# gbbin/DDP-practice

Hardware: AMD Instinct MI355X
Metric: images/sec (whole node) + 3-epoch wall-clock, MNIST ConvNet at 1/2/4/8 MI355X (higher is better)
Workload: dtype bf16; 1 GPU; model=ConvNet (2x[Conv5x5-BN-ReLU-MaxPool2] + Linear(1568,10), 29,034 params), global_batch=32, parallelism=dp1, per_rank_batch=32, impl=native (fused HIP kernels, C++ reducer/communicator), sync_bn=False, amp=autocast bf16 + GradScaler, optimizer=SGD(lr=1e-4), hipgraph=True, steps_per_graph=16, comm=none (1 rank), grad_avg=none (1 rank)

## Files before the change

ddp_practice_amd/csrc/kernels/convblock_impl.h:

```cpp
#pragma once
#include "common.h"
#include "comm/xsite.h"

namespace dpa {
namespace cb {

constexpr int NTHR = 256;

__host__ __device__ constexpr int stats_len(int C) { return 3 * C + 1; }
__host__ __device__ constexpr int fslab_row(int C) { return 2 * C + 1; }

template <int I> struct SH;
template <> struct SH<0> { static constexpr int CIN = 1, COUT = 16, H = 28, W = 28, SPLIT = 4, WROWS = 28; };
#ifndef DPA_FWD2_SPLIT
#define DPA_FWD2_SPLIT 2
#endif
template <> struct SH<1> { static constexpr int CIN = 16, COUT = 32, H = 14, W = 14, SPLIT = DPA_FWD2_SPLIT, WROWS = 14; };
constexpr int kBwdSplit = 8;

template <int N, typename Sink>
__device__ __forceinline__ void stage_f32(const float* __restrict__ src, Sink&& sink) {
  static_assert(N % 4 == 0, "N must be a multiple of 4");
  constexpr int N4 = N / 4;
  constexpr int IT = (N4 + NTHR - 1) / NTHR;
  f32x4 v[IT];
  const f32x4* s4 = reinterpret_cast<const f32x4*>(src);
#pragma unroll
  for (int i = 0; i < IT; ++i) {
    const int e = threadIdx.x + i * NTHR;
    if (e < N4) v[i] = s4[e];
  }
#pragma unroll
  for (int i = 0; i < IT; ++i) {
    const int e = threadIdx.x + i * NTHR;
    if (e < N4) {
#pragma unroll
      for (int j = 0; j < 4; ++j) sink(4 * e + j, v[i][j]);
    }
  }
}

template <typename T> struct Pair2 { typedef uint32_t type; };
template <> struct Pair2<float> { typedef uint64_t type; };
template <typename T, int C, int H, int W, typename Sink>
__device__ __forceinline__ void stage_chw(const T* __restrict__ src, Sink&& sink) {
  static_assert(W % 2 == 0, "W must be even");
  typedef typename Pair2<T>::type P;
  constexpr int NP = C * H * W / 2;
  constexpr int IT = (NP + NTHR - 1) / NTHR;
  P v[IT];
  const P* s2 = reinterpret_cast<const P*>(src);
#pragma unroll
  for (int i = 0; i < IT; ++i) {
    const int e = threadIdx.x + i * NTHR;
    if (e < NP) v[i] = s2[e];
  }
#pragma unroll
  for (int i = 0; i < IT; ++i) {
    const int e = threadIdx.x + i * NTHR;
    if (e < NP) {
      const int pe = 2 * e;
      const int c = pe / (H * W), rem = pe % (H * W);
      T a, b;
      __builtin_memcpy(&a, &v[i], sizeof(T));
      __builtin_memcpy(&b, reinterpret_cast<const char*>(&v[i]) + sizeof(T), sizeof(T));
      sink(c, rem / W, rem % W, a, b);
    }
  }
}

struct BNParams {
  const float* fslab;
  int nrows;
  float* fstats;
  const float* gamma;
  const float* beta;
  float* rmean;
  float* rvar;
  int64_t* nbt;
  float momentum;
  float eps;
  int train;
  xgmi::XSite xs;
};

constexpr int RSUM_U = 24;
template <typename F>
__device__ __forceinline__ float strided_rowsum(const float* __restrict__ src, int rows, int RL, int j, int g, int G,
                                                F&& after_issue) {
  float acc = 0.f;
  auto batch = [&](int base, bool first) {
    float v[RSUM_U];
#pragma unroll
    for (int u = 0; u < RSUM_U; ++u) {
      const int rr = base + u * G;
      v[u] = src[(size_t)min(rr, rows - 1) * RL + j] * (rr < rows ? 1.f : 0.f);
    }
    if (first) after_issue();
#pragma unroll
    for (int u = 0; u < RSUM_U; ++u) acc += v[u];
  };
  batch(g, true);
  for (int base = g + RSUM_U * G; base < rows; base += RSUM_U * G) batch(base, false);
  return acc;
}
__device__ __forceinline__ float strided_rowsum(const float* __restrict__ src, int rows, int RL, int j, int g, int G) {
  return strided_rowsum(src, rows, RL, j, g, G, [] {});
}

template <int C>
__device__ __forceinline__ void bn_finalize(const BNParams& bp, float* sc_s, float* beta_s, float* mean_s,
                                            float* istd_s, float* part, int bid) {
  const int tid = threadIdx.x, nthr = NTHR;
  const bool leader = bid == 0;
  if (bp.train) {
    constexpr int RL = 2 * C + 1;
    const int G = nthr / RL;
    const int j = tid % RL, g = tid / RL;
    float gam = 0.f, bet = 0.f, shf = 0.f, rm = 0.f, rv = 0.f;
    if (tid < C) {
      gam = bp.gamma[tid];
      bet = bp.beta[tid];
      shf = bp.fstats[2 * C + 1 + tid];
      if (leader) {
        rm = bp.rmean[tid];
        rv = bp.rvar[tid];
      }
    }
    const int64_t nb0 = leader ? bp.nbt[0] : 0;
    const bool xon = bp.xs.active();
    unsigned long long tk = 0;
    auto ticket = [&] {
      if (xon && tid == 0) tk = xgmi::xsite_ticket(bp.xs, bid);
    };
    if (g < G) {
      part[tid] = strided_rowsum(bp.fslab, bp.nrows, RL, j, g, G, ticket);
    } else {
      ticket();
      part[tid] = 0.f;
    }
    DPA_STAMP(11);
    __syncthreads();
    DPA_STAMP(12);
    if (tid < RL) {
      float t = 0.f;
      for (int gg = 0; gg < G; ++gg) t += part[gg * RL + tid];
      part[tid] = t;
    }
    __syncthreads();
    if (xon) xgmi::xsite_exchange(bp.xs, part, RL, tk, bid);
    if (tid < C) {
      const float n = part[2 * C];
      const float m1 = part[tid] / n;
      const float mean = shf + m1;
      const float var = fmaxf(part[C + tid] / n - m1 * m1, 0.f);
      const float istd = rsqrtf(var + bp.eps);
      const float s = gam * istd;
      sc_s[tid] = s;
      beta_s[tid] = bet;
      mean_s[tid] = mean;
      istd_s[tid] = istd;
      if (leader) {
        bp.fstats[tid] = part[tid];
        bp.fstats[C + tid] = part[C + tid];
        if (tid == 0) bp.fstats[2 * C] = n;
        const int64_t nb = nb0 + 1;
        const float mom = bp.momentum >= 0.f ? bp.momentum : 1.f / (float)nb;
        bp.rmean[tid] = (1.f - mom) * rm + mom * mean;
        bp.rvar[tid] = (1.f - mom) * rv + mom * var * (n / fmaxf(n - 1.f, 1.f));
      }
    }
    __syncthreads();
    if (leader && tid == 0) bp.nbt[0] = nb0 + 1;
  } else {
    if (tid < C) {
      const float istd = rsqrtf(bp.rvar[tid] + bp.eps);
      const float s = bp.gamma[tid] * istd;
      sc_s[tid] = s;
      beta_s[tid] = bp.beta[tid];
      mean_s[tid] = bp.rmean[tid];
      istd_s[tid] = istd;
    }
    __syncthreads();
  }
}

template <typename T>
__device__ __forceinline__ void bn_relu_max4x(const typename Pair2<T>::type top, const typename Pair2<T>::type bot,
                                              float sc, float beta, float mean, float istd, float& best, int& bi,
                                              float& xh) {
  T v[4];
  __builtin_memcpy(&v[0], &top, 2 * sizeof(T));
  __builtin_memcpy(&v[2], &bot, 2 * sizeof(T));
  best = -1.f;
  bi = 0;
  float yb = 0.f;
#pragma unroll
  for (int k = 0; k < 4; ++k) {
    const float yv = Cvt<T>::to_f(v[k]);
    const float z = fmaxf(rnd_t<T>((yv - mean) * sc + beta), 0.f);
    if (z > best) { best = z; bi = k; yb = yv; }
  }
  xh = (yb - mean) * istd;
}

constexpr int IDX_POS = 3, IDX_RELU = 4;

template <typename T>
struct PoolIn {
  const T* y;
  BNParams bn;
  T* p_out;
  uint8_t* idx_out;
  T* xh_out;
};

template <typename T>
struct BwdIn {
  const T* dp;
  const uint8_t* idx;
  const T* y;
  const float* fstats;
  const float* gsum;
  int grows;
  const float* lsum;
  int lrows;
  const float* gamma;
  float eps;
  float* dgamma;
  float* dbeta;
  xgmi::XSite xs;
  GradChk chk;
  int chk_coef = 0;
  int chk_rows = 0;
  float chk_row_bound = 0.f;
};

__device__ __forceinline__ void colsum_rows(const float* __restrict__ src, int rows, int RL, float* part,
                                            float* out) {
  const int tid = threadIdx.x, nthr = NTHR;
  const int G = nthr / RL;
  const int j = tid % RL, g = tid / RL;
  part[tid] = g < G ? strided_rowsum(src, rows, RL, j, g, G) : 0.f;
  __syncthreads();
  float t = 0.f;
  if (tid < RL)
    for (int gg = 0; gg < G; ++gg) t += part[gg * RL + tid];
  __syncthreads();
  if (tid < RL) out[tid] = t;
  __syncthreads();
}

template <int C, typename T>
__device__ __forceinline__ void bn_bwd_coef(const BwdIn<T>& bi, float* coef, float* part, float* sums, int bid) {
  const int tid = threadIdx.x;
  const bool leader = bid == 0;
  float n = 0.f, f0 = 0.f, f1 = 0.f, shf = 0.f, gam = 0.f;
  if (tid < C) {
    n = bi.fstats[2 * C];
    f0 = bi.fstats[tid];
    f1 = bi.fstats[C + tid];
    shf = bi.fstats[2 * C + 1 + tid];
    gam = bi.gamma[tid];
  }
  const bool xon = bi.xs.active();
  unsigned long long tk = 0;
  if (xon && tid == 0) tk = xgmi::xsite_ticket(bi.xs, bid);
  const bool cchk = leader && bi.dgamma != nullptr && bi.chk_coef && !xon;
  colsum_rows(bi.gsum, bi.grows, 2 * C, part, sums);
  if (xon) {
    if (leader && bi.dgamma != nullptr && tid < C) {
      bi.dgamma[tid] = sums[C + tid];
      bi.dbeta[tid] = sums[tid];
      if (bi.chk_coef) bi.chk.flag(GradChk::bad(sums[C + tid], bi.chk.bound) || GradChk::bad(sums[tid], bi.chk.bound));
    }
    xgmi::xsite_exchange(bi.xs, sums, 2 * C, tk, bid);
  }
  if (tid < C) {
    const float m1 = f0 / n;
    const float mean = shf + m1;
    const float istd = rsqrtf(fmaxf(f1 / n - m1 * m1, 0.f) + bi.eps);
    coef[tid] = sums[tid] / n;
    coef[C + tid] = sums[C + tid] / n;
    coef[2 * C + tid] = gam * istd;
    coef[3 * C + tid] = mean;
    coef[4 * C + tid] = istd;
    if (leader && bi.dgamma != nullptr && bi.lsum == bi.gsum && !xon) {
      bi.dgamma[tid] = sums[C + tid];
      bi.dbeta[tid] = sums[tid];
    }
  }
  __syncthreads();
  if (leader && bi.dgamma != nullptr && bi.lsum != bi.gsum && !xon) {
    colsum_rows(bi.lsum, bi.lrows, 2 * C, part, sums);
    if (tid < C) {
      bi.dgamma[tid] = sums[C + tid];
      bi.dbeta[tid] = sums[tid];
    }
  }
  if (cchk && tid < C)
    bi.chk.flag(GradChk::bad(sums[C + tid], bi.chk.bound) || GradChk::bad(sums[tid], bi.chk.bound));
}

template <typename T, int C, int H, int W, int NT_, int ROWS = H>
struct BnBwdStage {
  typedef typename Pair2<T>::type P;
  static_assert(ROWS % 2 == 0 && ROWS <= H, "BN-backward staging works on whole 2x2 pooling windows");
  static constexpr int HO = H / 2, WO = W / 2, PP = HO * WO;
  static constexpr int CHO = ROWS / 2, CPP = CHO * WO, NWIN = C * CPP;
  static constexpr int IT = (NWIN + NT_ - 1) / NT_;
// ... 214 lines not shown
      return px * CIN + c;
    } else {
      return px * CIN + ((((c >> 3) ^ ((px / PPB) & (NCH - 1)))) << 3) + (c & 7);
    }
  };
  __shared__ float lstat[(NTHR / 64) * 2 * COUT];

  const int tid = threadIdx.x;
  const int b = bid / nsplit;
  DPA_STAMP(0);
  const int sp = bid % nsplit;
  const T* xb = x + (size_t)b * CIN * HW;
  const int mt0 = (MT * sp) / nsplit, mt1 = (MT * (sp + 1)) / nsplit;
  float pre_bias[NT], pre_shift[NT];
#pragma unroll
  for (int nt = 0; nt < NT; ++nt) {
    const int co = nt * 16 + (tid & 15);
    pre_bias[nt] = (MODE == 2) ? 0.f : bias[co];
    pre_shift[nt] = (MODE == 0) ? shift[co] : 0.f;
  }

  const T zero = Cvt<T>::from_f(0.f);
  constexpr int WN16 = WPK == 1 ? COUT * KPW * (int)sizeof(T) / 16 : 1;
  constexpr int WIT = (WN16 + NTHR - 1) / NTHR;
  auto load_wpk = [&]() {
    if constexpr (WPK == 1) {
      static_assert((COUT * KPW * sizeof(T)) % 16 == 0, "packed weight tile must be whole 16-B chunks");
      static_assert(COUT * KPW == (MODE == 2 ? W2D_LEN : W2F_LEN), "pre-packed weights exist for layer 2 only");
      typedef __attribute__((address_space(3))) void* lds_ptr_t;
      const uint4* src = reinterpret_cast<const uint4*>(wpk);
      uint4* dstl = reinterpret_cast<uint4*>(wl);
      const int wv0 = (tid >> 6) * 64, ln = tid & 63;
#pragma unroll
      for (int i = 0; i < WIT; ++i) {
        const int c0 = i * NTHR + wv0;
        if (c0 + ln < WN16)
          __builtin_amdgcn_global_load_lds(src + c0 + ln, (lds_ptr_t)(dstl + c0), 16, 0, 0);
      }
    }
  };
  if constexpr (WPK == 1) {
    if constexpr (PRO == 0 || PRO == 3) load_wpk();
  } else {
    if constexpr (KP > K) {
      for (int e = tid; e < COUT * (KP - K); e += NTHR) wl[(e / (KP - K)) * KPW + K + e % (KP - K)] = zero;
    }
    constexpr int KO = 25 * (MODE == 2 ? COUT : CIN);
    stage_f32<COUT * K>(w, [&](int e, float v) {
      const int o = e / KO, rem = e % KO;
      const int i = rem / 25, tap = rem % 25;
      if (MODE == 2)
        wl[i * KPW + (24 - tap) * CIN + o] = Cvt<T>::from_f(v);
      else
        wl[o * KPW + tap * CIN + i] = Cvt<T>::from_f(v);
    });
  }
  if constexpr (WPK == 2) pack_w2<T>(pk);
  DPA_STAMP(1);
  if constexpr ((CIN * sizeof(T)) % 16 == 0) {
    constexpr int G = CIN * (int)sizeof(T) / 16;
    uint4* img4 = reinterpret_cast<uint4*>(img);
    for (int e = tid; e < HP * WPD * G; e += NTHR) {
      const int px = e / G, hp = px / WPD, wp = px % WPD;
      if (hp < 2 || hp >= H + 2 || wp < 2 || wp >= W + 2) img4[e] = make_uint4(0u, 0u, 0u, 0u);
    }
  } else {
    for (int e = tid; e < HP * WPD * CIN; e += NTHR) {
      const int hp = e / (WPD * CIN), rem = e % (WPD * CIN);
      const int wp = rem / CIN;
      if (hp < 2 || hp >= H + 2 || wp < 2 || wp >= W + 2) img[e] = zero;
    }
  }
  constexpr int EPIX = EPI ? MT * 16 : 1;
  __shared__ uint8_t eidx[EPI ? COUT * EPIX : 1];
  __shared__ T exh[EPI ? COUT * EPIX : 1];
  const int ep0 = mt0 * 16, enp = min(mt1 * 16, HW) - ep0;
  constexpr int EIT = EPI ? (COUT * EPIX + NTHR - 1) / NTHR : 1;
  uint8_t ei[EIT];
  T ex[EIT];
  auto load_epi = [&]() {
    if constexpr (EPI == 1) {
#pragma unroll
      for (int i = 0; i < EIT; ++i) {
        const int e = tid + i * NTHR;
        const int ec = e < COUT * enp ? e : 0;
        const int co = ec / enp, pp = ec % enp;
        const size_t o = ((size_t)b * COUT + co) * HW + ep0 + pp;
        ei[i] = epi.idx[o];
        ex[i] = epi.xh[o];
      }
    }
  };
  auto store_epi = [&]() {
    if constexpr (EPI == 1) {
#pragma unroll
      for (int i = 0; i < EIT; ++i) {
        const int e = tid + i * NTHR;
        if (e < COUT * enp) {
          const int co = e / enp, pp = e % enp;
          eidx[co * EPIX + pp] = ei[i];
          exh[co * EPIX + pp] = ex[i];
        }
      }
    }
  };
  if constexpr (PRO != 2) {
    load_epi();
    store_epi();
  }
  DPA_STAMP(2);
  constexpr int DQ = PRO != 1 ? 1
                     : (CIN % 8 == 0 && sizeof(T) == 2) ? 8 * ((CIN / 8 * HW + NTHR - 1) / NTHR)
                                                          : (CIN * HW + NTHR - 1) / NTHR;
  int dq_e[DQ];
  T dq_p[DQ], dq_x[DQ];
  uint8_t dq_i[DQ];
#pragma unroll
  for (int d = 0; d < DQ; ++d) dq_e[d] = -1;
  if constexpr (PRO == 0) {
    stage_chw<T, CIN, H, W>(xb, [&](int ci, int h, int ww, T a, T bb) {
      img[imo((h + 2) * WPD + (ww + 2), ci)] = a;
      img[imo((h + 2) * WPD + (ww + 3), ci)] = bb;
    });
  } else if constexpr (PRO == 3) {
    static_assert(HW % 4 == 0 && W % 4 == 0, "4-pixel groups stay inside a row");
    constexpr int G4 = HW / 4, GIT = (G4 + NTHR - 1) / NTHR;
    const int step = __builtin_amdgcn_readfirstlane(*reinterpret_cast<volatile int*>(gin.ctr));
    long long pos = (long long)step * gin.nimg + b;
    pos = pos < gin.order_len ? pos : gin.order_len - 1;
    const int64_t src = gin.order[pos];
    const uint32_t* s4 = reinterpret_cast<const uint32_t*>(gin.imgs + src * HW);
    uint32_t v4[GIT];
#pragma unroll
    for (int i = 0; i < GIT; ++i)
      if (tid + i * NTHR < G4) v4[i] = s4[tid + i * NTHR];
    if (sp == 0 && tid == 0) gin.lab_out[b] = gin.labels[src];
    T* xo = const_cast<T*>(xb);
#pragma unroll
    for (int i = 0; i < GIT; ++i) {
      const int g = tid + i * NTHR;
      if (g < G4) {
        const int h = (4 * g) / W, ww = (4 * g) % W;
        T px[4];
#pragma unroll
        for (int k = 0; k < 4; ++k) {
          px[k] = Cvt<T>::from_f((float)((v4[i] >> (8 * k)) & 0xffu) * gin.scale + gin.shift);
          img[imo((h + 2) * WPD + (ww + k + 2), 0)] = px[k];
        }
        if (sp == 0) {
#pragma unroll
          for (int k = 0; k < 4; ++k) xo[4 * g + k] = px[k];
        }
      }
    }
    if (tid == 0) {
      const int arrived = __hip_atomic_fetch_add(&gin.ctr[1], 1, __ATOMIC_RELAXED, __HIP_MEMORY_SCOPE_AGENT);
      if (arrived == gin.nimg * nsplit - 1) {
        __hip_atomic_store(&gin.ctr[1], 0, __ATOMIC_RELAXED, __HIP_MEMORY_SCOPE_AGENT);
        __hip_atomic_store(&gin.ctr[0], step + 1, __ATOMIC_RELAXED, __HIP_MEMORY_SCOPE_AGENT);
      }
    }
  } else if constexpr (PRO == 1) {
    __shared__ float sc_s[CIN], beta_s[CIN], mean_s[CIN], istd_s[CIN];
    __shared__ float part[NTHR];
    typedef typename Pair2<T>::type P;
    constexpr int NPO = CIN * HW;
    const T* yb = pin.y + (size_t)b * CIN * 4 * HW;
    const bool wr = pin.p_out != nullptr;
    const int e_lo = NPO * sp / nsplit, e_hi = NPO * (sp + 1) / nsplit;
    if constexpr (CIN % 8 == 0 && sizeof(T) == 2) {
      constexpr int NO = CIN / 8, NPI = NO * HW, IT8 = (NPI + NTHR - 1) / NTHR;
      P top[IT8][8], bot[IT8][8];
#pragma unroll
      for (int i = 0; i < IT8; ++i) {
        const int e8 = tid + i * NTHR;
        if (e8 < NPI) {
          const int o = e8 / HW, pix = e8 % HW, ho = pix / W, wo = pix % W;
#pragma unroll
          for (int j = 0; j < 8; ++j) {
            const P* src =
                reinterpret_cast<const P*>(yb + ((size_t)(8 * o + j) * 2 * H + 2 * ho) * 2 * W + 2 * wo);
            top[i][j] = src[0];
            bot[i][j] = src[W];
          }
        }
      }
      load_wpk();
      bn_finalize<CIN>(pin.bn, sc_s, beta_s, mean_s, istd_s, part, bid);
      DPA_STAMP(3);
#pragma unroll
      for (int i = 0; i < IT8; ++i) {
        const int e8 = tid + i * NTHR;
        if (e8 < NPI) {
          const int o = e8 / HW, pix = e8 % HW, ho = pix / W, wo = pix % W;
          unsigned pk[4];
#pragma unroll
          for (int j = 0; j < 8; ++j) {
            const int ci = 8 * o + j;
            float best, xh;
            int bi;
            bn_relu_max4x<T>(top[i][j], bot[i][j], sc_s[ci], beta_s[ci], mean_s[ci], istd_s[ci], best, bi, xh);
            const T pvj = Cvt<T>::from_f(best);
            const unsigned bits = __builtin_bit_cast(unsigned short, pvj);
            if (j & 1) pk[j >> 1] |= bits << 16; else pk[j >> 1] = bits;
            const int e = ci * HW + pix;
            const int d = i * 8 + j;
            dq_e[d] = wr && e >= e_lo && e < e_hi ? e : -1;
            dq_p[d] = pvj;
            dq_i[d] = (uint8_t)(bi | (best > 0.f ? IDX_RELU : 0));
            dq_x[d] = Cvt<T>::from_f(xh);
          }
          *reinterpret_cast<uint4*>(&img[imo((ho + 2) * WPD + (wo + 2), 8 * o)]) = make_uint4(pk[0], pk[1], pk[2], pk[3]);
        }
      }
    } else {
      constexpr int IT = (NPO + NTHR - 1) / NTHR;
      P top[IT], bot[IT];
#pragma unroll
      for (int i = 0; i < IT; ++i) {
        const int e = tid + i * NTHR;
        if (e < NPO) {
          const int ci = e / HW, pix = e % HW, ho = pix / W, wo = pix % W;
          const P* src = reinterpret_cast<const P*>(yb + ((size_t)ci * 2 * H + 2 * ho) * 2 * W + 2 * wo);
          top[i] = src[0];
          bot[i] = src[W];
        }
      }
      load_wpk();
      bn_finalize<CIN>(pin.bn, sc_s, beta_s, mean_s, istd_s, part, bid);
      DPA_STAMP(3);
#pragma unroll
      for (int i = 0; i < IT; ++i) {
        const int e = tid + i * NTHR;
        if (e < NPO) {
          const int ci = e / HW, pix = e % HW, ho = pix / W, wo = pix % W;
          float best, xh;
          int bi;
          bn_relu_max4x<T>(top[i], bot[i], sc_s[ci], beta_s[ci], mean_s[ci], istd_s[ci], best, bi, xh);
          const T pv = Cvt<T>::from_f(best);
          img[imo((ho + 2) * WPD + (wo + 2), ci)] = pv;
          dq_e[i] = wr && e >= e_lo && e < e_hi ? e : -1;
          dq_p[i] = pv;
          dq_i[i] = (uint8_t)(bi | (best > 0.f ? IDX_RELU : 0));
          dq_x[i] = Cvt<T>::from_f(xh);
        }
      }
    }
  } else {
    __shared__ float coef[5 * CIN], sums[2 * CIN];
    __shared__ float part[NTHR];
    if constexpr (CIN % 8 == 0 && sizeof(T) == 2) {
      BnBwdStage8<T, CIN, H, W, NTHR> st;
      st.load(bin, b);
      DPA_STAMP(8);
      load_wpk();
      bn_bwd_coef<CIN, T>(bin, coef, part, sums, bid);
      load_epi();
      DPA_STAMP(3);
      st.emit(coef, [&](int h, int ww, int c0, uint4 q00, uint4 q01, uint4 q10, uint4 q11) {
        *reinterpret_cast<uint4*>(&img[imo((h + 2) * WPD + (ww + 2), c0)]) = q00;
        *reinterpret_cast<uint4*>(&img[imo((h + 2) * WPD + (ww + 3), c0)]) = q01;
        *reinterpret_cast<uint4*>(&img[imo((h + 3) * WPD + (ww + 2), c0)]) = q10;
        *reinterpret_cast<uint4*>(&img[imo((h + 3) * WPD + (ww + 3), c0)]) = q11;
      });
    } else {
      BnBwdStage<T, CIN, H, W, NTHR> st;
      st.load(bin, b);
      DPA_STAMP(8);
      load_wpk();
      bn_bwd_coef<CIN, T>(bin, coef, part, sums, bid);
      load_epi();
      DPA_STAMP(3);
      st.emit(coef, [&](int c, int h, int ww, T v00, T v01, T v10, T v11) {
        img[imo((h + 2) * WPD + (ww + 2), c)] = v00;
        img[imo((h + 2) * WPD + (ww + 3), c)] = v01;
        img[imo((h + 3) * WPD + (ww + 2), c)] = v10;
        img[imo((h + 3) * WPD + (ww + 3), c)] = v11;
      });
    }
    store_epi();
  }
  DPA_STAMP(4);
  __syncthreads();
  DPA_STAMP(5);
  if constexpr (PRO == 1) {
    constexpr int NPO = CIN * HW;
#pragma unroll
    for (int d = 0; d < DQ; ++d)
      if (dq_e[d] >= 0) {
        const size_t o = (size_t)b * NPO + dq_e[d];
        pin.p_out[o] = dq_p[d];
        pin.idx_out[o] = dq_i[d];
        pin.xh_out[o] = dq_x[d];
      }
  }

  const int lane = tid & 63, wv = tid >> 6;
  const int r = lane & 15, q = lane >> 4;

  float s1[NT], s2[NT];
#pragma unroll
  for (int nt = 0; nt < NT; ++nt) s1[nt] = s2[nt] = 0.f;

  for (int mt = mt0 + wv; mt < mt1; mt += NTHR / 64) {
    const int m = mt * 16 + r;
    const int mm_ = m < HW ? m : HW - 1;
    const int oh = mm_ / W, ow = mm_ % W;
    f32x4 acc[NT];
#pragma unroll
    for (int nt = 0; nt < NT; ++nt) acc[nt] = f32x4{0.f, 0.f, 0.f, 0.f};
#pragma unroll
    for (int s = 0; s < KS; ++s) {
      typename mm::frag a;
      if constexpr (CIN == 1) {
#pragma unroll
        for (int j = 0; j < 8; ++j) {
          const int tap = 32 * s + 8 * q + j;
          float v = 0.f;
          if (tap < 25) v = Cvt<T>::to_f(img[(oh + tap / 5) * WPD + ow + tap % 5]);
          a[j] = mm::cv(v);
        }
      } else {
        const int kb = 32 * s + 8 * q;
        int tap = kb / CIN;
        const int ci0 = kb % CIN;
        tap = tap < 25 ? tap : 24;
        a = mm::ld(&img[imo((oh + tap / 5) * WPD + ow + tap % 5, ci0)]);
      }
#pragma unroll
      for (int nt = 0; nt < NT; ++nt) {
        const typename mm::frag bf = mm::ld(&wl[(nt * 16 + r) * KPW + 32 * s + 8 * q]);
        acc[nt] = mm::mma(a, bf, acc[nt]);
      }
    }
    const int pix0 = mt * 16 + 4 * q;
    if (pix0 < HW) {
#pragma unroll
      for (int nt = 0; nt < NT; ++nt) {
        const int co = nt * 16 + r;
        const float bs = pre_bias[nt];
        T* dst = y + ((size_t)b * COUT + co) * HW + pix0;
        const float sh = pre_shift[nt];
#pragma unroll
        for (int i = 0; i < 4; ++i) {
          const float v = acc[nt][i] + bs;
          dst[i] = Cvt<T>::from_f(v);
          if (MODE == 0) {
            const float d = rnd_t<T>(v) - sh;
            s1[nt] += d;
            s2[nt] += d * d;
          }
          if (EPI == 1) {
            const int le = co * EPIX + pix0 - mt0 * 16 + i;
            const float g = (eidx[le] & IDX_RELU) ? rnd_t<T>(v) : 0.f;
            s1[nt] += g;
            s2[nt] += g * Cvt<T>::to_f(exh[le]);
          }
        }
      }
    }
  }
  DPA_STAMP(6);
  if constexpr (MODE == 0 || EPI == 1) {
#pragma unroll
    for (int nt = 0; nt < NT; ++nt) {
      const float a1 = xor32_sum(xor16_sum(s1[nt])), a2 = xor32_sum(xor16_sum(s2[nt]));
      if (q == 0) {
        lstat[wv * 2 * COUT + nt * 16 + r] = a1;
        lstat[wv * 2 * COUT + COUT + nt * 16 + r] = a2;
      }
    }
    __syncthreads();
    float* row = (MODE == 0 ? fslab + (size_t)bid * fslab_row(COUT)
                            : epi.bslab + (size_t)bid * 2 * COUT);
    if (tid < 2 * COUT) {
      float t = 0.f;
#pragma unroll
      for (int w2 = 0; w2 < NTHR / 64; ++w2) t += lstat[w2 * 2 * COUT + tid];
      row[tid] = t;
    }
    if constexpr (MODE == 0) {
      if (tid == 0) {
        const int p0 = mt0 * 16, p1 = min(mt1 * 16, HW);
        row[2 * COUT] = (float)(p1 - p0);
      }
      if (bid == 0 && tid < COUT) fstats[2 * COUT + 1 + tid] = shift[tid];
    }
  }
  DPA_STAMP(7);
}

template <typename T, int CIN, int COUT, int H, int W, int MODE, int PRO = 0, int EPI = 0, int WPK = 0>
__global__ void __launch_bounds__(NTHR)
conv5x5_kernel(const T* __restrict__ x, const float* __restrict__ w, const float* __restrict__ bias,
               T* __restrict__ y, float* __restrict__ fslab, float* __restrict__ fstats,
               const float* __restrict__ shift, int nsplit, PoolIn<T> pin = PoolIn<T>{},
               BwdIn<T> bin = BwdIn<T>{}, BwdEpi<T> epi = BwdEpi<T>{}, const T* __restrict__ wpk = nullptr,
               WPack<T> pk = WPack<T>{}, GatherIn gin = GatherIn{}) {
  conv5x5_body<T, CIN, COUT, H, W, MODE, PRO, EPI, WPK>(x, w, bias, y, fslab, fstats, shift, nsplit, pin, bin, epi,
                                                        wpk, pk, (int)blockIdx.x, gin);
}

template <typename T, int C, int H, int W>
__global__ void __launch_bounds__(NTHR)
bn_relu_pool_kernel(const T* __restrict__ y, const float* __restrict__ fslab, int nrows,
                    float* __restrict__ fstats, const float* __restrict__ gamma, const float* __restrict__ beta,
                    float* __restrict__ rmean, float* __restrict__ rvar, int64_t* __restrict__ nbt,
                    float momentum, float eps, int train, T* __restrict__ p, uint8_t* __restrict__ idx,
                    int total) {
  constexpr int HO = H / 2, WO = W / 2;
  constexpr int RL = 2 * C + 1;
  __shared__ float part[NTHR];
  __shared__ float sc_s[C], beta_s[C], mean_s[C];
  const int tid = threadIdx.x;
  if (train) {
    constexpr int G = NTHR / RL;
    static_assert(G >= 1, "C too large");
    const int j = tid % RL, g = tid / RL;
    float a0 = 0.f, a1 = 0.f, a2 = 0.f, a3 = 0.f;
    if (g < G) {
      int rr = g;
      for (; rr + 3 * G < nrows; rr += 4 * G) {
        a0 += fslab[(size_t)rr * RL + j];
        a1 += fslab[(size_t)(rr + G) * RL + j];
        a2 += fslab[(size_t)(rr + 2 * G) * RL + j];
        a3 += fslab[(size_t)(rr + 3 * G) * RL + j];
      }
      for (; rr < nrows; rr += G) a0 += fslab[(size_t)rr * RL + j];
    }
    part[tid] = (a0 + a1) + (a2 + a3);
    __syncthreads();
    if (tid < RL) {
      float t = 0.f;
      for (int gg = 0; gg < G; ++gg) t += part[gg * RL + tid];
      part[tid] = t;
    }
    __syncthreads();
    if (tid < C) {
      const float n = part[2 * C];
      const float m1 = part[tid] / n;
      const float shv = fstats[2 * C + 1 + tid];
      const float mean = shv + m1;
      const float var = fmaxf(part[C + tid] / n - m1 * m1, 0.f);
      const float invstd = rsqrtf(var + eps);
      const float s = gamma[tid] * invstd;
      sc_s[tid] = s;
      beta_s[tid] = beta[tid];
      mean_s[tid] = mean;
      if (blockIdx.x == 0) {
        fstats[tid] = part[tid];
        fstats[C + tid] = part[C + tid];
        if (tid == 0) fstats[2 * C] = n;
        const int64_t nb = nbt[0] + 1;
        const float mom = momentum >= 0.f ? momentum : 1.f / (float)nb;
        rmean[tid] = (1.f - mom) * rmean[tid] + mom * mean;
        rvar[tid] = (1.f - mom) * rvar[tid] + mom * var * (n / fmaxf(n - 1.f, 1.f));
      }
    }
    __syncthreads();
    if (blockIdx.x == 0 && tid == 0) nbt[0] = nbt[0] + 1;
  } else {
    if (tid < C) {
      const float invstd = rsqrtf(rvar[tid] + eps);
      const float s = gamma[tid] * invstd;
      sc_s[tid] = s;
      beta_s[tid] = beta[tid];
      mean_s[tid] = rmean[tid];
    }
    __syncthreads();
  }
  const int e = blockIdx.x * NTHR + tid;
  if (e >= total) return;
  const int c = (e / (HO * WO)) % C;
  const float sc = sc_s[c], bt = beta_s[c], mn = mean_s[c];
  const int bc = e / (HO * WO), pix = e % (HO * WO);
  const int ho = pix / WO, wo = pix % WO;
  const T* src = y + (size_t)bc * H * W + (2 * ho) * W + 2 * wo;
  float best = -1.f;
  int bi = 0;
#pragma unroll
  for (int k = 0; k < 4; ++k) {
    const float v = Cvt<T>::to_f(src[(k >> 1) * W + (k & 1)]);
    const float z = fmaxf(rnd_t<T>((v - mn) * sc + bt), 0.f);
    if (z > best) { best = z; bi = k; }
  }
  p[e] = Cvt<T>::from_f(best);
  idx[e] = (uint8_t)bi;
}

template <int C>
__device__ __forceinline__ void stats_mean_invstd(const float* fstats, int c, float eps, float& mean,
                                                  float& invstd, float& n) {
  n = fstats[2 * C];
  const float m1 = fstats[c] / n;
  mean = fstats[2 * C + 1 + c] + m1;
  invstd = rsqrtf(fmaxf(fstats[C + c] / n - m1 * m1, 0.f) + eps);
}

template <typename T, int C, int H, int W>
__global__ void __launch_bounds__(NTHR)
bwd_reduce_kernel(const T* __restrict__ dp, const T* __restrict__ p, const uint8_t* __restrict__ idx,
                  const T* __restrict__ y, const float* __restrict__ fstats, float eps,
                  float* __restrict__ bslab, int B) {
  constexpr int HO = H / 2, WO = W / 2, PP = HO * WO;
  __shared__ float red[2 * NTHR / 64];
  const int c = blockIdx.x;
  const int nsplit = gridDim.y;
  const int b0 = (B * blockIdx.y) / nsplit, b1 = (B * (blockIdx.y + 1)) / nsplit;
  float mean, invstd, n;
  stats_mean_invstd<C>(fstats, c, eps, mean, invstd, n);
  float a1 = 0.f, a2 = 0.f;
  const int cnt = (b1 - b0) * PP;
  for (int t = threadIdx.x; t < cnt; t += NTHR) {
    const int b = b0 + t / PP, pix = t % PP;
    const size_t e = ((size_t)b * C + c) * PP + pix;
    const float pv = Cvt<T>::to_f(p[e]);
    if (pv > 0.f) {
      const float g = Cvt<T>::to_f(dp[e]);
      const int k = idx[e];
      const int ho = pix / WO, wo = pix % WO;
      const float yv = Cvt<T>::to_f(
          y[((size_t)b * C + c) * H * W + (2 * ho + (k >> 1)) * W + 2 * wo + (k & 1)]);
      a1 += g;
      a2 += g * (yv - mean) * invstd;
    }
  }
  a1 = wave_sum(a1);
  a2 = wave_sum(a2);
  const int lane = threadIdx.x & 63, wv = threadIdx.x >> 6;
  if (lane == 0) { red[wv] = a1; red[NTHR / 64 + wv] = a2; }
  __syncthreads();
  if (threadIdx.x == 0) {
    float t1 = 0.f, t2 = 0.f;
    for (int i = 0; i < NTHR / 64; ++i) { t1 += red[i]; t2 += red[NTHR / 64 + i]; }
    bslab[blockIdx.y * 2 * C + c] = t1;
    bslab[blockIdx.y * 2 * C + C + c] = t2;
  }
}

template <typename T, int C, int H, int W>
__global__ void __launch_bounds__(NTHR)
bwd_elemt_kernel(const T* __restrict__ dp, const T* __restrict__ p, const uint8_t* __restrict__ idx,
                 const T* __restrict__ y, const float* __restrict__ fstats,
                 const float* __restrict__ gslab, int nsplit, const float* __restrict__ gamma, float eps,
                 T* __restrict__ dx, int total) {
  constexpr int HO = H / 2, WO = W / 2, PP = HO * WO;
  __shared__ float k_s[3 * C];
  __shared__ float m_s[2 * C];
  const int tid = threadIdx.x;
  if (tid < C) {
    float s1 = 0.f, s2 = 0.f;
    for (int s = 0; s < nsplit; ++s) {
      s1 += gslab[s * 2 * C + tid];
      s2 += gslab[s * 2 * C + C + tid];
    }
    float mean, invstd, n;
    stats_mean_invstd<C>(fstats, tid, eps, mean, invstd, n);
    k_s[tid] = s1 / n;
    k_s[C + tid] = s2 / n;
    k_s[2 * C + tid] = gamma[tid] * invstd;
    m_s[tid] = mean;
    m_s[C + tid] = invstd;
  }
  __syncthreads();
  const int e = blockIdx.x * NTHR + tid;
  if (e >= total) return;
  const int bc = e / PP, pix = e % PP;
  const int c = bc % C;
  const float k1 = k_s[c], k2 = k_s[C + c], gi = k_s[2 * C + c];
  const float mean = m_s[c], invstd = m_s[C + c];
  const float pv = Cvt<T>::to_f(p[e]);
  const float g = pv > 0.f ? Cvt<T>::to_f(dp[e]) : 0.f;
  const int kk = idx[e];
  const int ho = pix / WO, wo = pix % WO;
  const size_t base = (size_t)bc * H * W + (2 * ho) * W + 2 * wo;
#pragma unroll
  for (int k = 0; k < 4; ++k) {
    const size_t o = base + (k >> 1) * W + (k & 1);
    const float xh = (Cvt<T>::to_f(y[o]) - mean) * invstd;
    const float dy = (k == kk) ? g : 0.f;
    dx[o] = Cvt<T>::from_f(gi * (dy - k1 - xh * k2));
  }
}

template <typename T, int CIN, int COUT, int H, int W, int ROWS>
struct WgradLds {
  static constexpr int WP = ceil_to(W, 8), XR = ROWS + 4, WX = WP + 4, N = CIN * 25;
  static constexpr int DYS = ROWS * WP + 8, XCS = XR * WP + 8;
  static constexpr bool DIRECT = ROWS == H, CIF = CIN >= 16;
  static constexpr size_t DYL = sizeof(T) * (size_t)COUT * DYS;
  static constexpr size_t XS = sizeof(T) * (size_t)5 * CIN * XCS;
  static constexpr size_t XPAD = sizeof(T) * (size_t)(DIRECT ? 8 : CIN * XR * WX);
  static constexpr size_t BASE = DYL + XS + XPAD;
  static constexpr bool STAGE = CIF && BASE + sizeof(float) * (size_t)COUT * N <= 144 * 1024;
  static constexpr size_t o_xs = (DYL + 15) / 16 * 16, o_xpad = (o_xs + XS + 15) / 16 * 16,
                          o_wt = (o_xpad + XPAD + 15) / 16 * 16;
  static constexpr size_t bytes = o_wt + sizeof(float) * (STAGE ? (size_t)COUT * N : 4);
};

template <typename T, int CIN, int COUT, int H, int W, int ROWS, int PRO = 0, bool WT = false, bool CHK = false,
          bool DYN = false>
__device__ __forceinline__ void
conv5x5_wgrad_body(const T* __restrict__ x, const T* __restrict__ dy, float* __restrict__ wslab, int nsplit,
                   const BwdIn<T>& bin, const int bid) {
  auto put = [](float* p, float v) {
    if constexpr (WT) __hip_atomic_store(p, v, __ATOMIC_RELAXED, __HIP_MEMORY_SCOPE_AGENT);
    else *p = v;
  };
  static_assert(PRO == 0 || (PRO == 2 && ROWS % 2 == 0), "PRO 2 works on whole 2x2 pooling windows");
  constexpr int WP = ceil_to(W, 8);
  static_assert((ROWS * WP) % 32 == 0, "ROWS*WP must be a multiple of 32");
  constexpr int KSTEPS = ROWS * WP / 32;
  constexpr int N = CIN * 25;
  constexpr int NTL = (N + 15) / 16;
  constexpr int MTL = COUT / 16;
  constexpr int PAIRS = MTL * NTL;
  constexpr int NW = NTHR / 64;
  constexpr int KSPLIT = PAIRS >= NW ? 1 : NW / PAIRS;
  constexpr int XR = ROWS + 4;
  constexpr int ROWLEN = COUT * N + COUT;
  typedef MM<T> mm;
  constexpr int DYS = ROWS * WP + 8;
  constexpr int XCS = XR * WP + 8;
  constexpr bool CIF = CIN >= 16;
  constexpr int WX = WP + 4;
  constexpr bool DIRECT = (ROWS == H);
  __shared__ f32x4 kred[KSPLIT > 1 ? NW : 1][64];
  using WL = WgradLds<T, CIN, COUT, H, W, ROWS>;
  constexpr bool STAGE = WL::STAGE;
  T* dyl;
  T* xs;
  T* xpad;
  float* wtile;
  if constexpr (DYN) {
    dyl = reinterpret_cast<T*>(dpa_dyn_lds);
    xs = reinterpret_cast<T*>(dpa_dyn_lds + WL::o_xs);
    xpad = reinterpret_cast<T*>(dpa_dyn_lds + WL::o_xpad);
    wtile = reinterpret_cast<float*>(dpa_dyn_lds + WL::o_wt);
  } else {
    __shared__ __attribute__((aligned(16))) T dyl_s[COUT * DYS];
    __shared__ __attribute__((aligned(16))) T xs_s[5 * CIN * XCS];
    __shared__ __attribute__((aligned(16))) T xpad_s[DIRECT ? 8 : CIN * XR * WX];
    __shared__ __attribute__((aligned(16))) float wtile_s[STAGE ? COUT * N : 4];
    dyl = dyl_s;
    xs = xs_s;
    xpad = xpad_s;
    wtile = wtile_s;
  }

  const int tid = threadIdx.x;
  const int b = bid / nsplit, sp = bid % nsplit;
  DPA_STAMP(0);
  const bool rchk = CHK && bin.chk_rows;
  const int r0 = sp * ROWS;
  const T* xb = x + (size_t)b * CIN * H * W;
  auto stage_xpad = [&]() {
    if constexpr (!DIRECT) {
      constexpr int XN = CIN * XR * W, XIT = (XN + NTHR - 1) / NTHR;
      T xv[XIT];
#pragma unroll
      for (int i = 0; i < XIT; ++i) {
        const int e = threadIdx.x + i * NTHR;
        const int ci = e / (XR * W), rem = e % (XR * W);
        const int rr = rem / W, cc = rem % W;
        const int ih = r0 + rr - 2;
        const bool ok = e < XN && ih >= 0 && ih < H;
        xv[i] = xb[ok ? (ci * H + ih) * W + cc : 0];
      }
#pragma unroll
      for (int i = 0; i < XIT; ++i) {
        const int e = threadIdx.x + i * NTHR;
        const int ci = e / (XR * W), rem = e % (XR * W);
        const int rr = rem / W, cc = rem % W;
        const int ih = r0 + rr - 2;
        if (e < XN && ih >= 0 && ih < H) xpad[(ci * XR + rr) * WX + cc + 2] = xv[i];
      }
    }
  };
  const T* dyb = dy + (size_t)b * COUT * H * W;
  const T zero = Cvt<T>::from_f(0.f);

  for (int e = tid; e < COUT * ROWS * (WP - W); e += NTHR) {
    const int cr = e / (WP - W), cc = W + e % (WP - W);
    dyl[(cr / ROWS) * DYS + (cr % ROWS) * WP + cc] = zero;
  }
  if (r0 + ROWS > H) {
    for (int e = tid; e < COUT * ROWS * WP; e += NTHR)
      if (r0 + (e / WP) % ROWS >= H) dyl[(e / (ROWS * WP)) * DYS + e % (ROWS * WP)] = zero;
  }
  auto scatter5 = [&](int ci, int rr, int w, T v) {
#pragma unroll
    for (int kw = 0; kw < 5; ++kw) {
      const int c = w + 2 - kw;
      if (c >= 0 && c < WP) xs[(kw * CIN + ci) * XCS + rr * WP + c] = v;
    }
  };
  if constexpr (DIRECT) {
    constexpr int NZ = 5 * CIN * XCS * (int)sizeof(T) / 16;
    static_assert((5 * CIN * XCS * sizeof(T)) % 16 == 0, "xs must be a whole number of 16-B chunks");
    uint4* z = reinterpret_cast<uint4*>(xs);
    for (int e = tid; e < NZ; e += NTHR) z[e] = make_uint4(0u, 0u, 0u, 0u);
  } else {
    for (int e = tid; e < CIN * XR * WX; e += NTHR) {
      const int cc = e % WX, rr = (e / WX) % XR;
      const int ih = r0 + rr - 2;
      if (cc < 2 || cc >= W + 2 || ih < 0 || ih >= H) xpad[e] = zero;
    }
  }
  if constexpr (PRO == 2) {
    __shared__ float coef[5 * COUT], sums[2 * COUT];
    __shared__ float part[NTHR];
    BnBwdStage<T, COUT, H, W, NTHR, ROWS> st;
    st.load(bin, b, r0);
    if constexpr (DIRECT) {
      __syncthreads();
      stage_chw<T, CIN, H, W>(xb, [&](int ci, int h, int ww, T a, T bb) {
        scatter5(ci, h + 2, ww, a);
        scatter5(ci, h + 2, ww + 1, bb);
      });
    } else {
      stage_xpad();
    }
    bn_bwd_coef<COUT, T>(bin, coef, part, sums, bid);
    DPA_STAMP(3);
    st.emit(coef, [&](int co, int h, int ww, T v00, T v01, T v10, T v11) {
      dyl[co * DYS + h * WP + ww] = v00;
      dyl[co * DYS + h * WP + ww + 1] = v01;
      dyl[co * DYS + (h + 1) * WP + ww] = v10;
      dyl[co * DYS + (h + 1) * WP + ww + 1] = v11;
    });
  } else if constexpr (DIRECT) {
    stage_chw<T, COUT, H, W>(dyb, [&](int co, int h, int ww, T a, T bb) {
      dyl[co * DYS + h * WP + ww] = a;
      dyl[co * DYS + h * WP + ww + 1] = bb;
    });
    __syncthreads();
    stage_chw<T, CIN, H, W>(xb, [&](int ci, int h, int ww, T a, T bb) {
      scatter5(ci, h + 2, ww, a);
      scatter5(ci, h + 2, ww + 1, bb);
    });
  } else {
    for (int e = tid; e < COUT * ROWS * W; e += NTHR) {
      const int co = e / (ROWS * W), rem = e % (ROWS * W);
      const int rr = rem / W, cc = rem % W;
      if (r0 + rr < H) dyl[co * DYS + rr * WP + cc] = dyb[(co * H + r0 + rr) * W + cc];
    }
    stage_xpad();
  }
  DPA_STAMP(4);
  __syncthreads();
  if constexpr (!DIRECT) {
    for (int e = tid; e < 5 * CIN * XR * (WP / 8); e += NTHR) {
      const int c8 = e % (WP / 8);
      const int rowid = e / (WP / 8);
      const int kw = rowid / (CIN * XR), cr = rowid % (CIN * XR);
      const T* srcp = &xpad[cr * WX + 8 * c8 + kw];
      T* dstp = &xs[(kw * CIN + cr / XR) * XCS + (cr % XR) * WP + 8 * c8];
#pragma unroll
      for (int j = 0; j < 8; ++j) dstp[j] = srcp[j];
    }
    __syncthreads();
  }

  float* row_out = wslab + (size_t)bid * ROWLEN;
  DPA_STAMP(5);
  const int lane = tid & 63, wv = tid >> 6;
  const int r = lane & 15, q = lane >> 4;
  {
    constexpr int TPC = NTHR / COUT;
    static_assert(NTHR % COUT == 0 && TPC <= 64 && (TPC & (TPC - 1)) == 0, "bias-sum lane groups");
    constexpr int E = ROWS * WP;
    static_assert(E % 8 == 0, "dy rows are whole 16-B groups");
    const int co = tid / TPC, sub = tid % TPC;
    float a = 0.f;
    for (int i = sub * 8; i < E; i += TPC * 8) {
      const typename mm::frag v = mm::ld(&dyl[co * DYS + i]);
      const T* e = reinterpret_cast<const T*>(&v);
#pragma unroll
      for (int j = 0; j < 8; ++j) a += Cvt<T>::to_f(e[j]);
    }
    a = group_sum<TPC>(a);
    if (sub == 0) {
      put(&row_out[COUT * N + co], a);
      if (rchk) bin.chk.flag(GradChk::bad(a, bin.chk_row_bound));
    }
  }
  DPA_STAMP(6);
  const int ks = KSPLIT > 1 ? wv % KSPLIT : 0;
  const int pstart = KSPLIT > 1 ? wv / KSPLIT : wv;
  const int pstep = KSPLIT > 1 ? NW / KSPLIT : NW;
  for (int pr = pstart; pr < PAIRS; pr += pstep) {
    const int mt = pr / NTL, nt = pr % NTL;
    int n = nt * 16 + r;
    n = n < N ? n : 0;
    const int ci = CIF ? n % CIN : n / 25, tap = CIF ? n / CIN : n % 25;
    const int kh = tap / 5, kw = tap % 5;
    const T* brow = &xs[(kw * CIN + ci) * XCS + kh * WP];
    const T* arow = &dyl[(mt * 16 + r) * DYS];
    f32x4 acc = {0.f, 0.f, 0.f, 0.f};
#pragma unroll
    for (int s = ks; s < KSTEPS; s += KSPLIT) {
      const int P = 32 * s + 8 * q;
      const int row = P / WP, col0 = P % WP;
      const typename mm::frag a = mm::ld(arow + P);
      const typename mm::frag bf = mm::ld(brow + row * WP + col0);
      acc = mm::mma(a, bf, acc);
    }
    if constexpr (KSPLIT > 1) {
      kred[wv][lane] = acc;
      __syncthreads();
      if (ks != 0) continue;
      for (int k2 = 1; k2 < KSPLIT; ++k2) acc += kred[wv + k2][lane];
    }
    const int col = nt * 16 + r;
    if (col < N) {
      const int nat = CIF ? (col % CIN) * 25 + col / CIN : col;
#pragma unroll
      for (int i = 0; i < 4; ++i) {
        if constexpr (STAGE) wtile[(mt * 16 + 4 * q + i) * N + nat] = acc[i];
        else put(&row_out[(mt * 16 + 4 * q + i) * N + nat], acc[i]);
        if (rchk) bin.chk.flag(GradChk::bad(acc[i], bin.chk_row_bound));
      }
    }
  }
  if constexpr (STAGE) {
    static_assert((COUT * N) % 4 == 0 && ROWLEN % 4 == 0, "wgrad rows: whole 16-B chunks");
    __syncthreads();
    if constexpr (WT) {
      for (int e = tid; e < COUT * N; e += NTHR) put(&row_out[e], wtile[e]);
    } else {
      for (int e = tid; e < COUT * N / 4; e += NTHR)
        *reinterpret_cast<f32x4*>(&row_out[4 * e]) = *reinterpret_cast<const f32x4*>(&wtile[4 * e]);
    }
  }
  DPA_STAMP(7);
}

template <typename T, int CIN, int COUT, int H, int W, int ROWS, int PRO = 0>
__global__ void __launch_bounds__(NTHR)
conv5x5_wgrad_kernel(const T* __restrict__ x, const T* __restrict__ dy, float* __restrict__ wslab,
                     int nsplit, BwdIn<T> bin = BwdIn<T>{}) {
  conv5x5_wgrad_body<T, CIN, COUT, H, W, ROWS, PRO>(x, dy, wslab, nsplit, bin, (int)blockIdx.x);
}

constexpr int SR_COLS = 16, SR_GROUPS = NTHR / SR_COLS;
__device__ __forceinline__ void slab_reduce_body(const float* __restrict__ slab1, int rows1, int n1,
                                                 float* __restrict__ out1, const float* __restrict__ slab2, int rows2,
                                                 int n2, float* __restrict__ out2, int bid,
                                                 GradChk chk = GradChk{}) {
  __shared__ float part[SR_GROUPS][SR_COLS + 1];
  const int nb1 = (n1 + SR_COLS - 1) / SR_COLS;
  const bool first = bid < nb1;
  const float* slab = first ? slab1 : slab2;
  const int rows = first ? rows1 : rows2;
  const int n = first ? n1 : n2;
  float* out = first ? out1 : out2;
  const int c0 = (first ? bid : bid - nb1) * SR_COLS;
  const int col = c0 + (threadIdx.x % SR_COLS), g = threadIdx.x / SR_COLS;
  part[g][threadIdx.x % SR_COLS] = slab_colsum<SR_GROUPS>(slab, rows, n, col, g);
  __syncthreads();
  if (threadIdx.x < SR_COLS && c0 + (int)threadIdx.x < n) {
    float t = 0.f;
#pragma unroll
    for (int gg = 0; gg < SR_GROUPS; ++gg) t += part[gg][threadIdx.x];
    out[c0 + threadIdx.x] = t;
    if (chk.word != nullptr) chk.flag(GradChk::bad(t, chk.bound));
  }
}
static __global__ void __launch_bounds__(NTHR)
slab_reduce_kernel(const float* __restrict__ slab1, int rows1, int n1, float* __restrict__ out1,
                   const float* __restrict__ slab2, int rows2, int n2, float* __restrict__ out2) {
  slab_reduce_body(slab1, rows1, n1, out1, slab2, rows2, n2, out2, (int)blockIdx.x);
}

}
}
```

Before: 663,200 images/s.

## Register-block conv MFMA loops: two M-tiles per wave, hoisted weights, mt-major wgrad

The forward conv tile loop for multi-channel inputs now has each wave process two M-tiles at once. For bf16 it hoists all weight fragments into registers and prefetches A fragments several K-steps ahead, with scheduling barriers. Addresses come from precomputed unsigned offsets. The wgrad kernel gains an mt-major path where each wave loads its dy fragments once and reuses them across several N-tiles, batching B loads. This cuts LDS traffic and index arithmetic but raises register pressure, and it changes the FMA contraction in the BN-stat accumulation.

```diff
diff --git a/ddp_practice_amd/csrc/kernels/convblock_impl.h b/ddp_practice_amd/csrc/kernels/convblock_impl.h
--- a/ddp_practice_amd/csrc/kernels/convblock_impl.h
+++ b/ddp_practice_amd/csrc/kernels/convblock_impl.h
@@ -1,4 +1,6 @@
 #pragma once
+#include <type_traits>
+
 #include "common.h"
 #include "comm/xsite.h"
 
@@ -6,6 +8,16 @@
 namespace cb {
 
 constexpr int NTHR = 256;
+
+template <bool FUSED>
+__device__ __forceinline__ float mul_add(float a, float b, float c) {
+  if constexpr (FUSED) {
+    return __builtin_fmaf(a, b, c);
+  } else {
+#pragma clang fp contract(off)
+    return a * b + c;
+  }
+}
 
 __host__ __device__ constexpr int stats_len(int C) { return 3 * C + 1; }
 __host__ __device__ constexpr int fslab_row(int C) { return 2 * C + 1; }
@@ -826,37 +838,8 @@
 #pragma unroll
   for (int nt = 0; nt < NT; ++nt) s1[nt] = s2[nt] = 0.f;
 
-  for (int mt = mt0 + wv; mt < mt1; mt += NTHR / 64) {
-    const int m = mt * 16 + r;
-    const int mm_ = m < HW ? m : HW - 1;
-    const int oh = mm_ / W, ow = mm_ % W;
-    f32x4 acc[NT];
-#pragma unroll
-    for (int nt = 0; nt < NT; ++nt) acc[nt] = f32x4{0.f, 0.f, 0.f, 0.f};
-#pragma unroll
-    for (int s = 0; s < KS; ++s) {
-      typename mm::frag a;
-      if constexpr (CIN == 1) {
-#pragma unroll
-        for (int j = 0; j < 8; ++j) {
-          const int tap = 32 * s + 8 * q + j;
-          float v = 0.f;
-          if (tap < 25) v = Cvt<T>::to_f(img[(oh + tap / 5) * WPD + ow + tap % 5]);
-          a[j] = mm::cv(v);
-        }
-      } else {
-        const int kb = 32 * s + 8 * q;
-        int tap = kb / CIN;
-        const int ci0 = kb % CIN;
-        tap = tap < 25 ? tap : 24;
-        a = mm::ld(&img[imo((oh + tap / 5) * WPD + ow + tap % 5, ci0)]);
-      }
-#pragma unroll
-      for (int nt = 0; nt < NT; ++nt) {
-        const typename mm::frag bf = mm::ld(&wl[(nt * 16 + r) * KPW + 32 * s + 8 * q]);
-        acc[nt] = mm::mma(a, bf, acc[nt]);
-      }
-    }
+  constexpr bool SQ_FUSED = sizeof(T) == 2;
+  auto epilogue = [&](const int mt, const f32x4 (&acc)[NT]) {
     const int pix0 = mt * 16 + 4 * q;
     if (pix0 < HW) {
 #pragma unroll
@@ -872,17 +855,136 @@
           if (MODE == 0) {
             const float d = rnd_t<T>(v) - sh;
             s1[nt] += d;
-            s2[nt] += d * d;
+            s2[nt] = mul_add<SQ_FUSED>(d, d, s2[nt]);
           }
           if (EPI == 1) {
             const int le = co * EPIX + pix0 - mt0 * 16 + i;
             const float g = (eidx[le] & IDX_RELU) ? rnd_t<T>(v) : 0.f;
             s1[nt] += g;
-            s2[nt] += g * Cvt<T>::to_f(exh[le]);
+            s2[nt] = mul_add<false>(g, Cvt<T>::to_f(exh[le]), s2[nt]);
           }
         }
       }
     }
+  };
+
+  if constexpr (CIN == 1) {
+    for (int mt = mt0 + wv; mt < mt1; mt += NTHR / 64) {
+      const int m = mt * 16 + r;
+      const int mm_ = m < HW ? m : HW - 1;
+      const int oh = mm_ / W, ow = mm_ % W;
+      f32x4 acc[NT];
+#pragma unroll
+      for (int nt = 0; nt < NT; ++nt) acc[nt] = f32x4{0.f, 0.f, 0.f, 0.f};
+#pragma unroll
+      for (int s = 0; s < KS; ++s) {
+        typename mm::frag a;
+#pragma unroll
+        for (int j = 0; j < 8; ++j) {
+          const int tap = 32 * s + 8 * q + j;
+          float v = 0.f;
+          if (tap < 25) v = Cvt<T>::to_f(img[(oh + tap / 5) * WPD + ow + tap % 5]);
+          a[j] = mm::cv(v);
+        }
+#pragma unroll
+        for (int nt = 0; nt < NT; ++nt) {
+          const typename mm::frag bf = mm::ld(&wl[(nt * 16 + r) * KPW + 32 * s + 8 * q]);
+          acc[nt] = mm::mma(a, bf, acc[nt]);
+        }
+      }
+      static_assert(EPI == 0, "the single-channel conv has no data-gradient epilogue");
+      const int pix0 = mt * 16 + 4 * q;
+      if (pix0 < HW) {
+#pragma unroll
+        for (int nt = 0; nt < NT; ++nt) {
+          const int co = nt * 16 + r;
+          const float bs = pre_bias[nt];
+          T* dst = y + ((size_t)b * COUT + co) * HW + pix0;
+          const float sh = pre_shift[nt];
+#pragma unroll
+          for (int i = 0; i < 4; ++i) {
+            const float v = acc[nt][i] + bs;
+            dst[i] = Cvt<T>::from_f(v);
+            if (MODE == 0) {
+              const float d = rnd_t<T>(v) - sh;
+              s1[nt] += d;
+              s2[nt] += d * d;
+            }
+          }
+        }
+      }
+    }
+  } else {
+    static_assert(CIN == 16 || CIN % 32 == 0, "tile loop: one or two taps per 32-deep K-step");
+    static_assert(NCH <= 16, "tile loop: a pixel is at most one 128-element bank row");
+    constexpr int NW = NTHR / 64;
+    constexpr int TPS = CIN < 32 ? 2 : 1;
+    constexpr bool BH = sizeof(T) == 2;
+    constexpr int AD = sizeof(T) == 2 ? (KS < 16 ? KS : 16) : 2;
+    const unsigned lane_ci = (8u * (unsigned)q) % CIN;
+    const unsigned lane_u = TPS == 2 ? (unsigned)q >> 1 : 0u;
+    auto tap_px = [](int tap) -> int {
+      tap = tap < 25 ? tap : 24;
+      return (tap / 5) * WPD + tap % 5;
+    };
+    typename mm::frag bh[BH ? KS : 1][NT];
+    if constexpr (BH) {
+#pragma unroll
+      for (int s = 0; s < KS; ++s)
+#pragma unroll
+        for (int nt = 0; nt < NT; ++nt) bh[s][nt] = mm::ld(&wl[(nt * 16 + r) * KPW + 32 * s + 8 * q]);
+    }
+    auto run_tiles = [&](auto ntc, const int mt) {
+      constexpr int NTI = decltype(ntc)::value;
+      unsigned b0[NTI], b1[NTI], b2[NTI];
+      f32x4 acc[NTI][NT];
+#pragma unroll
+      for (int t = 0; t < NTI; ++t) {
+        const unsigned m = (unsigned)(mt + t * NW) * 16u + (unsigned)r;
+        const unsigned mm_ = m < (unsigned)HW ? m : (unsigned)(HW - 1);
+        const unsigned oh = mm_ / (unsigned)W, ow = mm_ % (unsigned)W;
+        b0[t] = (oh * WPD + ow) * CIN + lane_ci;
+        b1[t] = b0[t] + lane_u * CIN;
+        b2[t] = b0[t] + lane_u * ((WPD - 4) * CIN);
+#pragma unroll
+        for (int nt = 0; nt < NT; ++nt) acc[t][nt] = f32x4{0.f, 0.f, 0.f, 0.f};
+      }
+      typename mm::frag a[NTI][KS];
+      auto read_a = [&](const int s) {
+        const int t0 = (32 * s) / CIN;
+        const int d = TPS == 2 ? tap_px(t0 + 1) - tap_px(t0) : 0;
+        const unsigned c = (unsigned)(tap_px(t0) * CIN + (32 * s) % CIN);
+#pragma unroll
+        for (int t = 0; t < NTI; ++t) {
+          const unsigned e = (d == 0 ? b0[t] : d == 1 ? b1[t] : b2[t]) + c;
+          if constexpr (NCH <= 1 || PAD8) a[t][s] = mm::ld(&img[e]);
+          else a[t][s] = mm::ld(&img[e ^ (((e >> 7) & (unsigned)(NCH - 1)) << 3)]);
+        }
+      };
+#pragma unroll
+      for (int s = 0; s < AD; ++s) read_a(s);
+      __builtin_amdgcn_sched_barrier(0);
+#pragma unroll
+      for (int s = 0; s < KS; ++s) {
+        if (s + AD < KS) {
+          read_a(s + AD);
+          __builtin_amdgcn_sched_barrier(0);
+        }
+#pragma unroll
+        for (int nt = 0; nt < NT; ++nt) {
+          typename mm::frag bf;
+          if constexpr (BH) bf = bh[s][nt];
+          else bf = mm::ld(&wl[(nt * 16 + r) * KPW + 32 * s + 8 * q]);
+#pragma unroll
+          for (int t = 0; t < NTI; ++t) acc[t][nt] = mm::mma(a[t][s], bf, acc[t][nt]);
+        }
+      }
+#pragma unroll
+      for (int t = 0; t < NTI; ++t) epilogue(mt + t * NW, acc[t]);
+    };
+    int mt = mt0 + wv;
+    for (; mt + NW < mt1; mt += 2 * NW) run_tiles(std::integral_constant<int, 2>{}, mt);
+    if (mt < mt1) run_tiles(std::integral_constant<int, 1>{}, mt);
   }
   DPA_STAMP(6);
   if constexpr (MODE == 0 || EPI == 1) {
@@ -1310,32 +1412,7 @@
     }
   }
   DPA_STAMP(6);
-  const int ks = KSPLIT > 1 ? wv % KSPLIT : 0;
-  const int pstart = KSPLIT > 1 ? wv / KSPLIT : wv;
-  const int pstep = KSPLIT > 1 ? NW / KSPLIT : NW;
-  for (int pr = pstart; pr < PAIRS; pr += pstep) {
-    const int mt = pr / NTL, nt = pr % NTL;
-    int n = nt * 16 + r;
-    n = n < N ? n : 0;
-    const int ci = CIF ? n % CIN : n / 25, tap = CIF ? n / CIN : n % 25;
-    const int kh = tap / 5, kw = tap % 5;
-    const T* brow = &xs[(kw * CIN + ci) * XCS + kh * WP];
-    const T* arow = &dyl[(mt * 16 + r) * DYS];
-    f32x4 acc = {0.f, 0.f, 0.f, 0.f};
-#pragma unroll
-    for (int s = ks; s < KSTEPS; s += KSPLIT) {
-      const int P = 32 * s + 8 * q;
-      const int row = P / WP, col0 = P % WP;
-      const typename mm::frag a = mm::ld(arow + P);
-      const typename mm::frag bf = mm::ld(brow + row * WP + col0);
-      acc = mm::mma(a, bf, acc);
-    }
-    if constexpr (KSPLIT > 1) {
-      kred[wv][lane] = acc;
-      __syncthreads();
-      if (ks != 0) continue;
-      for (int k2 = 1; k2 < KSPLIT; ++k2) acc += kred[wv + k2][lane];
-    }
+  auto store_pair = [&](const int mt, const int nt, const f32x4 acc) {
     const int col = nt * 16 + r;
     if (col < N) {
       const int nat = CIF ? (col % CIN) * 25 + col / CIN : col;
@@ -1345,6 +1422,81 @@
         else put(&row_out[(mt * 16 + 4 * q + i) * N + nat], acc[i]);
         if (rchk) bin.chk.flag(GradChk::bad(acc[i], bin.chk_row_bound));
       }
+    }
+  };
+  constexpr bool MTMAJOR = KSPLIT == 1 && CIF && CIN % 16 == 0 && N % 16 == 0 && NW % MTL == 0;
+  if constexpr (MTMAJOR) {
+    constexpr int WPM = NW / MTL;
+    constexpr int NTW = (NTL + WPM - 1) / WPM;
+    constexpr int FV = (int)sizeof(typename mm::frag) / 4;
+    constexpr int GMAX = 128 / (KSTEPS * FV) > 0 ? 128 / (KSTEPS * FV) : 1;
+    constexpr int G = NTW < GMAX ? NTW : GMAX;
+    constexpr int TPC = CIN / 16;
+    const int wvu = __builtin_amdgcn_readfirstlane(wv);
+    const int mt = wvu / WPM, nt0 = wvu % WPM;
+    typename mm::frag af[KSTEPS];
+#pragma unroll
+    for (int s = 0; s < KSTEPS; ++s) af[s] = mm::ld(&dyl[(mt * 16 + r) * DYS + 32 * s + 8 * q]);
+    const T* blane = &xs[r * XCS + 8 * q];
+    int tap = nt0 / TPC, cb0 = (nt0 % TPC) * 16;
+    int kh = tap / 5, kw = tap % 5;
+#pragma unroll
+    for (int g0 = 0; g0 < NTW; g0 += G) {
+      typename mm::frag bf[G][KSTEPS];
+#pragma unroll
+      for (int j = 0; j < G; ++j) {
+        if (g0 + j < NTW) {
+          const int khc = kh < 5 ? kh : 4, kwc = kh < 5 ? kw : 4;
+          const T* brow = blane + ((kwc * CIN + cb0) * XCS + khc * WP);
+#pragma unroll
+          for (int s = 0; s < KSTEPS; ++s) bf[j][s] = mm::ld(brow + 32 * s);
+          cb0 += (WPM % TPC) * 16;
+          kw += WPM / TPC + (cb0 >= CIN ? 1 : 0);
+          cb0 -= cb0 >= CIN ? CIN : 0;
+          kh += kw >= 5 ? 1 : 0;
+          kw -= kw >= 5 ? 5 : 0;
+        }
+      }
+      __builtin_amdgcn_sched_barrier(0);
+#pragma unroll
+      for (int j = 0; j < G; ++j) {
+        const int nt = nt0 + (g0 + j) * WPM;
+        if (g0 + j < NTW && nt < NTL) {
+          f32x4 acc = {0.f, 0.f, 0.f, 0.f};
+#pragma unroll
+          for (int s = 0; s < KSTEPS; ++s) acc = mm::mma(af[s], bf[j][s], acc);
+          store_pair(mt, nt, acc);
+        }
+      }
+    }
+  } else {
+    const int ks = KSPLIT > 1 ? wv % KSPLIT : 0;
+    const int pstart = KSPLIT > 1 ? wv / KSPLIT : wv;
+    const int pstep = KSPLIT > 1 ? NW / KSPLIT : NW;
+    for (int pr = pstart; pr < PAIRS; pr += pstep) {
+      const int mt = pr / NTL, nt = pr % NTL;
+      int n = nt * 16 + r;
+      n = n < N ? n : 0;
+      const int ci = CIF ? n % CIN : n / 25, tap = CIF ? n / CIN : n % 25;
+      const int kh = tap / 5, kw = tap % 5;
+      const T* brow = &xs[(kw * CIN + ci) * XCS + kh * WP];
+      const T* arow = &dyl[(mt * 16 + r) * DYS];
+      f32x4 acc = {0.f, 0.f, 0.f, 0.f};
+#pragma unroll
+      for (int s = ks; s < KSTEPS; s += KSPLIT) {
+        const int P = 32 * s + 8 * q;
+        const int row = P / WP, col0 = P % WP;
+        const typename mm::frag a = mm::ld(arow + P);
+        const typename mm::frag bf = mm::ld(brow + row * WP + col0);
+        acc = mm::mma(a, bf, acc);
+      }
+      if constexpr (KSPLIT > 1) {
+        kred[wv][lane] = acc;
+        __syncthreads();
+        if (ks != 0) continue;
+        for (int k2 = 1; k2 < KSPLIT; ++k2) acc += kred[wv + k2][lane];
+      }
+      store_pair(mt, nt, acc);
     }
   }
   if constexpr (STAGE) {
```

After: 660,000 images/s. Within noise of the previous version (-0.5%).
